# Gadersd/stable-diffusion-xl-burn

Measured on NVIDIA H100. Metric: unet_sampler_steps_per_sec_1024x1024_bs1, higher is better.
Workload: dtype f16

## Files before the change

stable-diffusion-xl-burn_b200/csrc/attention.cu:

```cuda
#include <stdlib.h>

#include "common.cuh"
#include "kernels.h"

namespace sdxl {

static constexpr int kTileBytes = 128 * 128;
static constexpr int kKvStages = 3;
static constexpr int kConsumerWarps = 8;
static constexpr int kAttnThreads = kConsumerWarps * 32 + 32;
static constexpr int kAttnSmem = 1024  + kTileBytes + 2 * kKvStages * kTileBytes + 256;

__device__ __forceinline__ float ex2_approx(float x) {
  float y;
  asm("ex2.approx.ftz.f32 %0, %1;" : "=f"(y) : "f"(x));
  return y;
}
__device__ __forceinline__ uint32_t pack_half2(float a, float b) {
  __half2 t = __floats2half2_rn(a, b);
  return *reinterpret_cast<uint32_t*>(&t);
}

__global__ void __launch_bounds__(kAttnThreads, 1) attention_kernel(const __grid_constant__ AttnParams p) {
  extern __shared__ uint8_t smem_raw[];
  uint8_t* smem = reinterpret_cast<uint8_t*>((reinterpret_cast<uintptr_t>(smem_raw) + 1023) & ~uintptr_t(1023));
  uint8_t* sQ = smem;
  uint8_t* sK = sQ + kTileBytes;
  uint8_t* sV = sK + kKvStages * kTileBytes;
  uint64_t* bars = reinterpret_cast<uint64_t*>(sV + kKvStages * kTileBytes);
  uint64_t* q_full = bars;
  uint64_t* kv_full = q_full + 1;
  uint64_t* kv_empty = kv_full + kKvStages;

  const int warp = threadIdx.x >> 5, lane = threadIdx.x & 31;
  const int nblk = (p.S + 127) / 128;
  const int nqt = (p.T + 127) / 128;
  const int qt = blockIdx.x % nqt, head = (blockIdx.x / nqt) % p.n_head, b = blockIdx.x / (nqt * p.n_head);

  if (threadIdx.x == 0) {
    tma_prefetch_desc(&p.tmQ);
    tma_prefetch_desc(&p.tmK);
    tma_prefetch_desc(&p.tmV);
    mbar_init(q_full, 1);
    for (int i = 0; i < kKvStages; ++i) { mbar_init(&kv_full[i], 1); mbar_init(&kv_empty[i], kConsumerWarps); }
    fence_barrier_init();
  }
  __syncthreads();
  griddep_wait();
  griddep_launch_dependents();

  if (warp == kConsumerWarps) {
    if (lane != 0) return;
    mbar_expect_tx(q_full, kTileBytes);
    tma_load_3d(sQ, &p.tmQ, q_full, p.q_col0 + head * 64, qt * 128, b);
    for (int j = 0; j < nblk; ++j) {
      const int st = j % kKvStages;
      mbar_wait_nocall(&kv_empty[st], ((j / kKvStages) & 1) ^ 1);
      mbar_expect_tx(&kv_full[st], 2 * kTileBytes);
      tma_load_3d(sK + st * kTileBytes, &p.tmK, &kv_full[st], p.k_col0 + head * 64, j * 128, b);
      tma_load_3d(sV + st * kTileBytes, &p.tmV, &kv_full[st], p.v_col0 + head * 64, j * 128, b);
    }
    return;
  }

  const int wg = warp >> 2;
  const float sl2e = p.scale_log2e;
  const uint32_t q_addr = smem_u32(sQ) + (uint32_t)wg * (64 * 128);
  float o[32];
#pragma unroll
  for (int i = 0; i < 32; ++i) o[i] = 0.f;
  float m[2] = {-INFINITY, -INFINITY}, l[2] = {0.f, 0.f};
  mbar_wait_nocall(q_full, 0);
  for (int j = 0; j < nblk; ++j) {
    const int st = j % kKvStages;
    mbar_wait_nocall(&kv_full[st], (j / kKvStages) & 1);
    float s[64];
    wg_fence();
    const uint32_t k_addr = smem_u32(sK + st * kTileBytes);
#pragma unroll
    for (int k = 0; k < 4; ++k) wgmma_ss_n128(s, wg_desc_sw128(q_addr + 32 * k), wg_desc_sw128(k_addr + 32 * k), k);
    wg_commit();
    wg_wait<0>();
    if (j * 128 + 128 > p.S) {
#pragma unroll
      for (int jj = 0; jj < 16; ++jj)
#pragma unroll
        for (int e = 0; e < 2; ++e)
          if (j * 128 + 8 * jj + 2 * (lane & 3) + e >= p.S) { s[4 * jj + e] = -INFINITY; s[4 * jj + 2 + e] = -INFINITY; }
    }
    uint32_t pa[32];
#pragma unroll
    for (int h = 0; h < 2; ++h) {
      float mx = -INFINITY;
#pragma unroll
      for (int jj = 0; jj < 16; ++jj) mx = fmaxf(mx, fmaxf(s[4 * jj + 2 * h], s[4 * jj + 2 * h + 1]));
      mx = fmaxf(mx, __shfl_xor_sync(0xffffffffu, mx, 1));
      mx = fmaxf(mx, __shfl_xor_sync(0xffffffffu, mx, 2));
      const float m_new = fmaxf(m[h], mx);
      const float alpha = ex2_approx((m[h] - m_new) * sl2e);
      const float mb = m_new * sl2e;
      float sum = 0.f;
#pragma unroll
      for (int jj = 0; jj < 16; ++jj) {
        const float p0 = ex2_approx(fmaf(s[4 * jj + 2 * h], sl2e, -mb));
        const float p1 = ex2_approx(fmaf(s[4 * jj + 2 * h + 1], sl2e, -mb));
        sum += p0 + p1;
        pa[4 * (jj >> 1) + 2 * (jj & 1) + h] = pack_half2(p0, p1);
      }
      l[h] = l[h] * alpha + sum;
      m[h] = m_new;
#pragma unroll
      for (int jj = 0; jj < 8; ++jj) { o[4 * jj + 2 * h] *= alpha; o[4 * jj + 2 * h + 1] *= alpha; }
    }
    wg_fence();
    const uint32_t v_addr = smem_u32(sV + st * kTileBytes);
#pragma unroll
    for (int kk = 0; kk < 8; ++kk)
      wgmma_rs_n64_tb(o, *reinterpret_cast<const uint32_t(*)[4]>(pa + 4 * kk), wg_desc_sw128(v_addr + 2048 * kk));
    wg_commit();
    wg_wait<0>();
    if (lane == 0) mbar_arrive(&kv_empty[st]);
  }
  const int r = wg * 64 + (warp & 3) * 16 + (lane >> 2);
#pragma unroll
  for (int h = 0; h < 2; ++h) {
    float lt = l[h];
    lt += __shfl_xor_sync(0xffffffffu, lt, 1);
    lt += __shfl_xor_sync(0xffffffffu, lt, 2);
    const float inv = 1.0f / lt;
    const int t = qt * 128 + r + 8 * h;
    if (t < p.T) {
      __half* out = p.out + ((size_t)b * p.T + t) * p.ldo + head * 64 + 2 * (lane & 3);
#pragma unroll
      for (int jj = 0; jj < 8; ++jj)
        *reinterpret_cast<__half2*>(out + 8 * jj) = __floats2half2_rn(o[4 * jj + 2 * h] * inv, o[4 * jj + 2 * h + 1] * inv);
    }
  }
}

static bool g_attn_attr[64];
int attention_launch(cudaStream_t st, const AttnParams& p) {
  if (p.T < 1 || p.S < 1 || (p.ldo & 1)) return 2002;
  int r = smem_optin(attention_kernel, kAttnSmem, g_attn_attr);
  if (r) return r;
  const long tiles = (long)p.B * p.n_head * ((p.T + 127) / 128);
  return launch_kernel(attention_kernel, dim3((unsigned)tiles), dim3(kAttnThreads), (size_t)kAttnSmem, st, true, p);
}

}
```

Measured before the change: 21.88.

## Make attention persistent with warp-specialized ping-pong and QK/PV software pipelining

```diff
diff --git a/stable-diffusion-xl-burn_b200/csrc/attention.cu b/stable-diffusion-xl-burn_b200/csrc/attention.cu
--- a/stable-diffusion-xl-burn_b200/csrc/attention.cu
+++ b/stable-diffusion-xl-burn_b200/csrc/attention.cu
@@ -8,8 +8,8 @@
 static constexpr int kTileBytes = 128 * 128;
 static constexpr int kKvStages = 3;
 static constexpr int kConsumerWarps = 8;
-static constexpr int kAttnThreads = kConsumerWarps * 32 + 32;
-static constexpr int kAttnSmem = 1024  + kTileBytes + 2 * kKvStages * kTileBytes + 256;
+static constexpr int kAttnThreads = 128 + kConsumerWarps * 32;
+static constexpr int kAttnSmem = 1024  + 2 * kTileBytes + 2 * kKvStages * kTileBytes + 256;
 
 __device__ __forceinline__ float ex2_approx(float x) {
   float y;
@@ -21,27 +21,100 @@
   return *reinterpret_cast<uint32_t*>(&t);
 }
 
+__device__ __forceinline__ void issue_qk(float (&s)[64], uint32_t q_addr, uint32_t k_addr) {
+#pragma unroll
+  for (int k = 0; k < 4; ++k) wgmma_ss_n128(s, wg_desc_sw128(q_addr + 32 * k), wg_desc_sw128(k_addr + 32 * k), k);
+  wg_commit();
+}
+__device__ __forceinline__ void issue_pv(float (&o)[32], const uint32_t (&pa)[32], uint32_t v_addr) {
+#pragma unroll
+  for (int kk = 0; kk < 8; ++kk)
+    wgmma_rs_n64_tb(o, *reinterpret_cast<const uint32_t(*)[4]>(pa + 4 * kk), wg_desc_sw128(v_addr + 2048 * kk));
+  wg_commit();
+}
+
+__device__ __forceinline__ void softmax_block(float (&s)[64], float (&m)[2], float (&l)[2], float (&alpha)[2], float sl2e,
+                                              int key0, int S, int lane) {
+  if (key0 + 128 > S) {
+#pragma unroll
+    for (int jj = 0; jj < 16; ++jj)
+#pragma unroll
+      for (int e = 0; e < 2; ++e)
+        if (key0 + 8 * jj + 2 * (lane & 3) + e >= S) { s[4 * jj + e] = -INFINITY; s[4 * jj + 2 + e] = -INFINITY; }
+  }
+#pragma unroll
+  for (int h = 0; h < 2; ++h) {
+    float mx = -INFINITY;
+#pragma unroll
+    for (int jj = 0; jj < 16; ++jj) mx = fmaxf(mx, fmaxf(s[4 * jj + 2 * h], s[4 * jj + 2 * h + 1]));
+    mx = fmaxf(mx, __shfl_xor_sync(0xffffffffu, mx, 1));
+    mx = fmaxf(mx, __shfl_xor_sync(0xffffffffu, mx, 2));
+    const float m_new = fmaxf(m[h], mx);
+    alpha[h] = ex2_approx((m[h] - m_new) * sl2e);
+    const float mb = m_new * sl2e;
+    float sum = 0.f;
+#pragma unroll
+    for (int jj = 0; jj < 16; ++jj) {
+      const float p0 = ex2_approx(fmaf(s[4 * jj + 2 * h], sl2e, -mb));
+      const float p1 = ex2_approx(fmaf(s[4 * jj + 2 * h + 1], sl2e, -mb));
+      sum += p0 + p1;
+      s[4 * jj + 2 * h] = p0;
+      s[4 * jj + 2 * h + 1] = p1;
+    }
+    l[h] = l[h] * alpha[h] + sum;
+    m[h] = m_new;
+  }
+}
+__device__ __forceinline__ void pack_p(const float (&s)[64], uint32_t (&pa)[32]) {
+#pragma unroll
+  for (int h = 0; h < 2; ++h)
+#pragma unroll
+    for (int jj = 0; jj < 16; ++jj) pa[4 * (jj >> 1) + 2 * (jj & 1) + h] = pack_half2(s[4 * jj + 2 * h], s[4 * jj + 2 * h + 1]);
+}
+__device__ __forceinline__ void rescale(float (&o)[32], const float (&alpha)[2]) {
+#pragma unroll
+  for (int h = 0; h < 2; ++h)
+#pragma unroll
+    for (int jj = 0; jj < 8; ++jj) { o[4 * jj + 2 * h] *= alpha[h]; o[4 * jj + 2 * h + 1] *= alpha[h]; }
+}
+template <int N>
+__device__ __forceinline__ void hold_regs(float (&r)[N]) {
+#pragma unroll
+  for (int i = 0; i < N; ++i) asm volatile("" : "+f"(r[i])::"memory");
+}
+template <int N>
+__device__ __forceinline__ void hold_regs(uint32_t (&r)[N]) {
+#pragma unroll
+  for (int i = 0; i < N; ++i) asm volatile("" : "+r"(r[i])::"memory");
+}
+__device__ __forceinline__ void wg_turn_wait(int wg) { asm volatile("bar.sync %0, 256;" ::"r"(1 + wg) : "memory"); }
+__device__ __forceinline__ void wg_turn_pass(int wg) { asm volatile("bar.arrive %0, 256;" ::"r"(2 - wg) : "memory"); }
+__device__ __forceinline__ void ring_next(uint32_t& stage, uint32_t& phase) {
+  if (++stage == (uint32_t)kKvStages) { stage = 0; phase ^= 1; }
+}
+
 __global__ void __launch_bounds__(kAttnThreads, 1) attention_kernel(const __grid_constant__ AttnParams p) {
   extern __shared__ uint8_t smem_raw[];
   uint8_t* smem = reinterpret_cast<uint8_t*>((reinterpret_cast<uintptr_t>(smem_raw) + 1023) & ~uintptr_t(1023));
   uint8_t* sQ = smem;
-  uint8_t* sK = sQ + kTileBytes;
+  uint8_t* sK = sQ + 2 * kTileBytes;
   uint8_t* sV = sK + kKvStages * kTileBytes;
   uint64_t* bars = reinterpret_cast<uint64_t*>(sV + kKvStages * kTileBytes);
   uint64_t* q_full = bars;
-  uint64_t* kv_full = q_full + 1;
+  uint64_t* q_empty = q_full + 2;
+  uint64_t* kv_full = q_empty + 2;
   uint64_t* kv_empty = kv_full + kKvStages;
 
   const int warp = threadIdx.x >> 5, lane = threadIdx.x & 31;
   const int nblk = (p.S + 127) / 128;
   const int nqt = (p.T + 127) / 128;
-  const int qt = blockIdx.x % nqt, head = (blockIdx.x / nqt) % p.n_head, b = blockIdx.x / (nqt * p.n_head);
+  const int ntiles = nqt * p.n_head * p.B;
 
   if (threadIdx.x == 0) {
     tma_prefetch_desc(&p.tmQ);
     tma_prefetch_desc(&p.tmK);
     tma_prefetch_desc(&p.tmV);
-    mbar_init(q_full, 1);
+    for (int i = 0; i < 2; ++i) { mbar_init(&q_full[i], 1); mbar_init(&q_empty[i], kConsumerWarps); }
     for (int i = 0; i < kKvStages; ++i) { mbar_init(&kv_full[i], 1); mbar_init(&kv_empty[i], kConsumerWarps); }
     fence_barrier_init();
   }
@@ -49,102 +122,126 @@
   griddep_wait();
   griddep_launch_dependents();
 
-  if (warp == kConsumerWarps) {
-    if (lane != 0) return;
-    mbar_expect_tx(q_full, kTileBytes);
-    tma_load_3d(sQ, &p.tmQ, q_full, p.q_col0 + head * 64, qt * 128, b);
-    for (int j = 0; j < nblk; ++j) {
-      const int st = j % kKvStages;
-      mbar_wait_nocall(&kv_empty[st], ((j / kKvStages) & 1) ^ 1);
-      mbar_expect_tx(&kv_full[st], 2 * kTileBytes);
-      tma_load_3d(sK + st * kTileBytes, &p.tmK, &kv_full[st], p.k_col0 + head * 64, j * 128, b);
-      tma_load_3d(sV + st * kTileBytes, &p.tmV, &kv_full[st], p.v_col0 + head * 64, j * 128, b);
+  if (warp < 4) {
+    setmaxnreg_dec<40>();
+    if (threadIdx.x != 0) return;
+    uint32_t stage = 0, phase = 0;
+    for (int tile = blockIdx.x, it = 0; tile < ntiles; tile += gridDim.x, ++it) {
+      const int qt = tile % nqt, head = (tile / nqt) % p.n_head, b = tile / (nqt * p.n_head);
+      const int qb = it & 1;
+      mbar_wait_nocall(&q_empty[qb], ((it >> 1) & 1) ^ 1);
+      mbar_expect_tx(&q_full[qb], kTileBytes);
+      tma_load_3d(sQ + qb * kTileBytes, &p.tmQ, &q_full[qb], p.q_col0 + head * 64, qt * 128, b);
+      for (int j = 0; j < nblk; ++j) {
+        mbar_wait_nocall(&kv_empty[stage], phase ^ 1);
+        mbar_expect_tx(&kv_full[stage], 2 * kTileBytes);
+        tma_load_3d(sK + stage * kTileBytes, &p.tmK, &kv_full[stage], p.k_col0 + head * 64, j * 128, b);
+        tma_load_3d(sV + stage * kTileBytes, &p.tmV, &kv_full[stage], p.v_col0 + head * 64, j * 128, b);
+        ring_next(stage, phase);
+      }
     }
     return;
   }
 
-  const int wg = warp >> 2;
+  setmaxnreg_inc<232>();
+  const int wg = (warp >> 2) - 1;
   const float sl2e = p.scale_log2e;
-  const uint32_t q_addr = smem_u32(sQ) + (uint32_t)wg * (64 * 128);
-  float o[32];
-#pragma unroll
-  for (int i = 0; i < 32; ++i) o[i] = 0.f;
-  float m[2] = {-INFINITY, -INFINITY}, l[2] = {0.f, 0.f};
-  mbar_wait_nocall(q_full, 0);
-  for (int j = 0; j < nblk; ++j) {
-    const int st = j % kKvStages;
-    mbar_wait_nocall(&kv_full[st], (j / kKvStages) & 1);
+  const uint32_t sK0 = smem_u32(sK), sV0 = smem_u32(sV);
+  uint32_t stage = 0, phase = 0;
+  if (wg == 1) wg_turn_pass(wg);
+  for (int tile = blockIdx.x, it = 0; tile < ntiles; tile += gridDim.x, ++it) {
+    const int qt = tile % nqt, head = (tile / nqt) % p.n_head, b = tile / (nqt * p.n_head);
+    const int qb = it & 1;
+    const uint32_t q_addr = smem_u32(sQ + qb * kTileBytes) + (uint32_t)wg * (64 * 128);
+    float o[32];
+#pragma unroll
+    for (int i = 0; i < 32; ++i) o[i] = 0.f;
+    float m[2] = {-INFINITY, -INFINITY}, l[2] = {0.f, 0.f}, alpha[2];
     float s[64];
+    uint32_t pa[32];
+    mbar_wait_nocall(&q_full[qb], (it >> 1) & 1);
+
+    mbar_wait_nocall(&kv_full[stage], phase);
+    wg_turn_wait(wg);
     wg_fence();
-    const uint32_t k_addr = smem_u32(sK + st * kTileBytes);
-#pragma unroll
-    for (int k = 0; k < 4; ++k) wgmma_ss_n128(s, wg_desc_sw128(q_addr + 32 * k), wg_desc_sw128(k_addr + 32 * k), k);
-    wg_commit();
+    issue_qk(s, q_addr, sK0 + stage * kTileBytes);
+    wg_turn_pass(wg);
     wg_wait<0>();
-    if (j * 128 + 128 > p.S) {
-#pragma unroll
-      for (int jj = 0; jj < 16; ++jj)
-#pragma unroll
-        for (int e = 0; e < 2; ++e)
-          if (j * 128 + 8 * jj + 2 * (lane & 3) + e >= p.S) { s[4 * jj + e] = -INFINITY; s[4 * jj + 2 + e] = -INFINITY; }
-    }
-    uint32_t pa[32];
+    hold_regs(s);
+    softmax_block(s, m, l, alpha, sl2e, 0, p.S, lane);
+    pack_p(s, pa);
+    rescale(o, alpha);
+    uint32_t prev = stage;
+    ring_next(stage, phase);
+
+    for (int j = 1; j < nblk; ++j) {
+      mbar_wait_nocall(&kv_full[stage], phase);
+      hold_regs(o);
+      hold_regs(pa);
+      wg_turn_wait(wg);
+      wg_fence();
+      issue_qk(s, q_addr, sK0 + stage * kTileBytes);
+      issue_pv(o, pa, sV0 + prev * kTileBytes);
+      wg_turn_pass(wg);
+      wg_wait<1>();
+      hold_regs(s);
+      softmax_block(s, m, l, alpha, sl2e, j * 128, p.S, lane);
+      hold_regs(s);
+      wg_wait<0>();
+      hold_regs(o);
+      hold_regs(pa);
+      if (lane == 0) mbar_arrive(&kv_empty[prev]);
+      pack_p(s, pa);
+      rescale(o, alpha);
+      prev = stage;
+      ring_next(stage, phase);
+    }
+    hold_regs(o);
+    hold_regs(pa);
+    wg_turn_wait(wg);
+    wg_fence();
+    issue_pv(o, pa, sV0 + prev * kTileBytes);
+    wg_turn_pass(wg);
+    wg_wait<0>();
+    hold_regs(o);
+    if (lane == 0) { mbar_arrive(&kv_empty[prev]); mbar_arrive(&q_empty[qb]); }
+
+    const int r = wg * 64 + (warp & 3) * 16 + (lane >> 2);
 #pragma unroll
     for (int h = 0; h < 2; ++h) {
-      float mx = -INFINITY;
-#pragma unroll
-      for (int jj = 0; jj < 16; ++jj) mx = fmaxf(mx, fmaxf(s[4 * jj + 2 * h], s[4 * jj + 2 * h + 1]));
-      mx = fmaxf(mx, __shfl_xor_sync(0xffffffffu, mx, 1));
-      mx = fmaxf(mx, __shfl_xor_sync(0xffffffffu, mx, 2));
-      const float m_new = fmaxf(m[h], mx);
-      const float alpha = ex2_approx((m[h] - m_new) * sl2e);
-      const float mb = m_new * sl2e;
-      float sum = 0.f;
-#pragma unroll
-      for (int jj = 0; jj < 16; ++jj) {
-        const float p0 = ex2_approx(fmaf(s[4 * jj + 2 * h], sl2e, -mb));
-        const float p1 = ex2_approx(fmaf(s[4 * jj + 2 * h + 1], sl2e, -mb));
-        sum += p0 + p1;
-        pa[4 * (jj >> 1) + 2 * (jj & 1) + h] = pack_half2(p0, p1);
+      float lt = l[h];
+      lt += __shfl_xor_sync(0xffffffffu, lt, 1);
+      lt += __shfl_xor_sync(0xffffffffu, lt, 2);
+      const float inv = 1.0f / lt;
+      const int t = qt * 128 + r + 8 * h;
+      if (t < p.T) {
+        __half* out = p.out + ((size_t)b * p.T + t) * p.ldo + head * 64 + 2 * (lane & 3);
+#pragma unroll
+        for (int jj = 0; jj < 8; ++jj)
+          *reinterpret_cast<__half2*>(out + 8 * jj) = __floats2half2_rn(o[4 * jj + 2 * h] * inv, o[4 * jj + 2 * h + 1] * inv);
       }
-      l[h] = l[h] * alpha + sum;
-      m[h] = m_new;
-#pragma unroll
-      for (int jj = 0; jj < 8; ++jj) { o[4 * jj + 2 * h] *= alpha; o[4 * jj + 2 * h + 1] *= alpha; }
-    }
-    wg_fence();
-    const uint32_t v_addr = smem_u32(sV + st * kTileBytes);
-#pragma unroll
-    for (int kk = 0; kk < 8; ++kk)
-      wgmma_rs_n64_tb(o, *reinterpret_cast<const uint32_t(*)[4]>(pa + 4 * kk), wg_desc_sw128(v_addr + 2048 * kk));
-    wg_commit();
-    wg_wait<0>();
-    if (lane == 0) mbar_arrive(&kv_empty[st]);
-  }
-  const int r = wg * 64 + (warp & 3) * 16 + (lane >> 2);
-#pragma unroll
-  for (int h = 0; h < 2; ++h) {
-    float lt = l[h];
-    lt += __shfl_xor_sync(0xffffffffu, lt, 1);
-    lt += __shfl_xor_sync(0xffffffffu, lt, 2);
-    const float inv = 1.0f / lt;
-    const int t = qt * 128 + r + 8 * h;
-    if (t < p.T) {
-      __half* out = p.out + ((size_t)b * p.T + t) * p.ldo + head * 64 + 2 * (lane & 3);
-#pragma unroll
-      for (int jj = 0; jj < 8; ++jj)
-        *reinterpret_cast<__half2*>(out + 8 * jj) = __floats2half2_rn(o[4 * jj + 2 * h] * inv, o[4 * jj + 2 * h + 1] * inv);
-    }
-  }
-}
-
-static bool g_attn_attr[64];
+    }
+  }
+  if (wg == 0) wg_turn_wait(wg);
+}
+
+struct AttnDev { bool attr = false; int num_sms = 0; };
+static AttnDev g_attn_dev[64];
 int attention_launch(cudaStream_t st, const AttnParams& p) {
   if (p.T < 1 || p.S < 1 || (p.ldo & 1)) return 2002;
-  int r = smem_optin(attention_kernel, kAttnSmem, g_attn_attr);
-  if (r) return r;
+  int dev = 0;
+  if (cudaGetDevice(&dev) != cudaSuccess || dev < 0 || dev >= 64) return 2001;
+  AttnDev& D = g_attn_dev[dev];
+  if (!D.attr) {
+    cudaError_t e = cudaFuncSetAttribute(attention_kernel, cudaFuncAttributeMaxDynamicSharedMemorySize, kAttnSmem);
+    if (e == cudaSuccess) e = cudaDeviceGetAttribute(&D.num_sms, cudaDevAttrMultiProcessorCount, dev);
+    if (e != cudaSuccess) return (int)e;
+    if (D.num_sms <= 0) D.num_sms = 132;
+    D.attr = true;
+  }
   const long tiles = (long)p.B * p.n_head * ((p.T + 127) / 128);
-  return launch_kernel(attention_kernel, dim3((unsigned)tiles), dim3(kAttnThreads), (size_t)kAttnSmem, st, true, p);
-}
-
-}
+  const unsigned grid = (unsigned)(tiles < D.num_sms ? tiles : D.num_sms);
+  return launch_kernel(attention_kernel, dim3(grid), dim3(kAttnThreads), (size_t)kAttnSmem, st, true, p);
+}
+
+}
```

Result: faster. 22.26 (median of 6 runs) (+1.7%).
